# quim0/WFA-GPU

Hardware: AMD Instinct MI355X
Metric: alignments_per_sec (higher is better)
Workload: dtype int32

## Files before the change

### wfa-gpu_amd/csrc/align/cells_hot.inc

```
      typedef __attribute__((address_space(3))) OffT* LdsRow;
      typedef __attribute__((address_space(3))) const uint32_t* LdsWords;
      typedef __attribute__((address_space(1))) uint8_t* GlobalBytes;
      typedef __attribute__((address_space(1))) OffT* GlobalRow;
      OffT* const hm_row0 = Mr + (dm + 2 * de) * rs + kidx0;
      auto hot_cells = [&](const int lo, const int wm1, GlobalBytes& codes, const uint32_t a_oe, const uint32_t a_x, const uint32_t a_m,
                           const uint32_t a_ip, const uint32_t a_ic, const uint32_t d_delta, const uint32_t pw_addr, const uint32_t tw_addr,
                           const uint32_t a_hm, unsigned long long& touch) {
        constexpr int SH = RAW ? 2 : 4, PER = 1 << SH, BITS = RAW ? 3 : 1;
        constexpr uint32_t TB = 16;
        constexpr bool PAIRED = HYBRID || BANDED;
        static_assert(TB >= (uint32_t)PER && (TB & (BT_M_MASK | BT_D_EXT | BT_I_EXT)) == 0, "tag base");
        auto group = [&](const int kq, const GlobalBytes codes, const int left) -> bool {
          bool more_groups;
          const uint32_t vb = (uint32_t)(kq - 1) << 1;
          const int kq16 = kq << 16;
          uint32_t q_mo = vb + a_oe, q_mx = vb + a_x, q_wm = vb + a_m, q_ri = vb + a_ip, q_wi = vb + a_ic;
          uint32_t q_rd = q_ri + d_delta, q_wd = q_wi + d_delta, q_hm = vb + a_hm;
          asm volatile("" : "+v"(q_mo), "+v"(q_mx), "+v"(q_wm), "+v"(q_ri), "+v"(q_wi), "+v"(q_rd), "+v"(q_wd), "+v"(q_hm));
          const LdsRow r_mo = (LdsRow)q_mo, r_mx = (LdsRow)q_mx, w_m = (LdsRow)q_wm;
          const LdsRow r_i = (LdsRow)q_ri, w_i = (LdsRow)q_wi, r_hm = (LdsRow)q_hm;
          auto d_row = [&](const uint32_t q) {
            if constexpr (HYBRID) return (GlobalRow)((GlobalBytes)(uintptr_t)d_first + (ptrdiff_t)(int32_t)q);
            else return (LdsRow)q;
          };
// ... 23 lines not shown
            asm("v_med3_i32 %0, %1, 0, %2" : "=v"(cap) : "v"(mv_t), "n"(PER));
            c.h = mv0;
            c.rem = c.hmax - c.h;
            if constexpr (!RAW) {
              const int vt = mv_t - kq16 - (O << 16);
              asm("v_lshl_add_u32 %0, %1, 2, %2" : "=v"(c.pa) : "v"(vt >> (16 + SH)), "s"(pw_addr));
              asm("v_lshl_add_u32 %0, %1, 2, %2" : "=v"(c.ta) : "v"(mv_t >> (16 + SH)), "s"(tw_addr));
              c.sa = (uint32_t)vt >> 15; c.sb = (uint32_t)mv_t >> 15;
            } else {
              const int v = mv0 - k;
              asm("v_lshl_add_u32 %0, %1, 2, %2" : "=v"(c.pa) : "v"(v >> SH), "s"(pw_addr));
              asm("v_lshl_add_u32 %0, %1, 2, %2" : "=v"(c.ta) : "v"(c.h >> SH), "s"(tw_addr));
              c.sa = (uint32_t)v << BITS; c.sb = (uint32_t)c.h << BITS;
            }
            uint32_t fb;
            {
              const LdsWords pw = (LdsWords)c.pa; const LdsWords tw = (LdsWords)c.ta;
              const uint32_t d0w = __builtin_amdgcn_alignbit(pw[1], pw[0], c.sa) ^ __builtin_amdgcn_alignbit(tw[1], tw[0], c.sb);
              asm("v_ffbl_b32 %0, %1" : "=v"(fb) : "v"(d0w));
            }
            int adv;
            asm("v_min3_i32 %0, %1, %2, %3" : "=v"(adv) : "v"((int)(fb >> BITS)), "v"(c.rem), "v"(cap));
            c.h += adv;
            c.more = adv == PER;
            return c;
          };
          auto back = [&](auto uc, auto partial_tag, const unsigned long long act, ChunkState& c) {
            constexpr int O = decltype(uc)::value * NT;
            constexpr bool PARTIAL = decltype(partial_tag)::value;
            if (__builtin_amdgcn_ballot_w64(c.more) != 0ull) {
              uint32_t fb;
              int togo = c.more ? max(c.rem - PER, 0) : 0;
              while (__builtin_amdgcn_ballot_w64(togo > 0) != 0ull) {
                c.pa += 4; c.ta += 4;
                const LdsWords pw = (LdsWords)c.pa; const LdsWords tw = (LdsWords)c.ta;
                const uint32_t d = __builtin_amdgcn_alignbit(pw[1], pw[0], c.sa) ^ __builtin_amdgcn_alignbit(tw[1], tw[0], c.sb);
                asm("v_ffbl_b32 %0, %1" : "=v"(fb) : "v"(d));
                const int nn = min(min((int)(fb >> BITS), PER), togo);
                c.h += nn;
                togo = (nn == PER) ? togo - PER : 0;
              }
            }
            int mv = c.h, ins_c = c.ins_c, del_t = c.del_t;
            if constexpr (PARTIAL) {
              const bool active = __builtin_amdgcn_inverse_ballot_w64(act);
              mv = active ? c.h : OffNull<OffT>::value;
              ins_c = active ? ins_c : (int)0x80000000u; del_t = active ? del_t : (int)0x80000000u;
            }
            touch |= __builtin_amdgcn_ballot_w64(mv == c.hmax);
            w_m[O + 1] = (OffT)mv;
            w_i[O + 1] = (OffT)(ins_c >> 16);
            w_d[O + 1] = (OffT)(del_t >> 16);
            if constexpr (BT) {
              if constexpr (TILED) codes[(size_t)(t_off + (uint32_t)(O * 4))] = (uint8_t)c.code;
              else codes[O] = (uint8_t)c.code;
            }
          };
          auto chunk = [&](auto uc, auto partial_tag, const unsigned long long act) {
            ChunkState c = front(uc);
            back(uc, partial_tag, act, c);
          };
          auto chunk_pair = [&](auto uc, auto uc2, auto partial2_tag, const unsigned long long act2) {
            ChunkState c0 = front(uc), c1 = front(uc2);
            back(uc, std::false_type{}, 0ull, c0);
            back(uc2, partial2_tag, act2, c1);
          };
          more_groups = false;
          auto from = [&](auto&& self, auto uc) -> void {
            constexpr int Uc = decltype(uc)::value;
            const int n_act = left - Uc * NT;
            if (n_act >= 64) {
              if constexpr (Uc < 3 && PAIRED) {
                const int n2 = n_act - NT;
                if (n2 >= 64) {
                  chunk_pair(uc, std::integral_constant<int, Uc + 1>{}, std::false_type{}, 0ull);
                  if constexpr (Uc + 1 < 3) { if (n2 > NT) self(self, std::integral_constant<int, Uc + 2>{}); }
                  else more_groups = n2 > NT;
                } else if (n2 > 0) {
                  chunk_pair(uc, std::integral_constant<int, Uc + 1>{}, std::true_type{}, (1ull << n2) - 1ull);
                } else {
                  chunk(uc, std::false_type{}, 0ull);
                }
              } else {
              chunk(uc, std::false_type{}, 0ull);
              if constexpr (Uc < 3) { if (n_act > NT) self(self, std::integral_constant<int, Uc + 1>{}); }
              else more_groups = n_act > NT;
              }
            } else if (NW == 1 || n_act > 0) {
              chunk(uc, std::true_type{}, (1ull << n_act) - 1ull);
            }
          };
          from(from, std::integral_constant<int, 0>{});
          return more_groups;
        };
        const int left0 = wm1 + 1 - ((NW == 1) ? 0 : __builtin_amdgcn_readfirstlane(stid & ~63));
        int kq = stid + lo, left = left0;
        if constexpr (NW == 1) {
          if (__builtin_expect(group(kq, codes, left), 0)) {
            constexpr uint32_t STEP = TILED ? 0u : 4u * NT;
            uint32_t adv = 0;
            do { kq += 4 * NT; codes += STEP; adv += STEP; left -= 4 * NT; } while (group(kq, codes, left));
            codes -= adv;
          }
        } else {
          uint32_t adv = 0;
          while (group(kq, codes, left)) { kq += 4 * NT; codes += 4 * NT; adv += 4u * NT; left -= 4 * NT; }
          codes -= adv;
// ... 3 lines not shown
```

### wfa-gpu_amd/csrc/align/loop_lean_any.inc

```
        if constexpr (HOT && !BANDED && !ENDSFREE) {
          if (e != 1 && !touched_ever) {
            const int s_in = s;
            const int o_pen = oe - e;
            int u_w = s_in >= oe ? (s_in - o_pen) / e : 0;
            int g_cnt = s_in >= oe ? e - (s_in - o_pen) % e : oe - s_in;
            int s_clear = INT_MAX;
            if (bounded) {
              const int lo_a = budget - e * (kend - wlo) + 1, lo_b = (budget + o_pen - e * (kend + 1)) / 2 + 1;
              const int hi_a = budget - e * (whi - kend) + 1, hi_b = (budget + o_pen + e * (kend - 1)) / 2 + 1;
              s_clear = min(min(lo_a, lo_b), min(hi_a, hi_b)) - 2 * e - 2;
            }
            s_clear = __builtin_amdgcn_readfirstlane(s_clear);
            const uint32_t rsb = (uint32_t)rs * 2u;
            const uint32_t a_first = lds_addr(m_first), a_end = lds_addr(m_end), ai_first = lds_addr(i_first), ai_end = lds_addr(i_end);
            uint32_t a_m = lds_addr(p_m), a_x = lds_addr(p_x), a_oe = lds_addr(p_oe), a_ic = lds_addr(p_ic), a_ip = lds_addr(p_ip);
            uint32_t d_delta = HYBRID ? 0u - ai_first : (uint32_t)(de * rs) * 2u;
            uint32_t pw_addr = lds_addr(Pw), tw_addr = lds_addr(Tw), a_hm = lds_addr(hm_row0);
            asm volatile("" : "+s"(pw_addr), "+s"(tw_addr), "+s"(a_hm), "+s"(d_delta));
            int lo = last_lo, hi = last_hi;
            int f_lo = max(wlo, rlo), f_hi = min(whi, rhi);
            unsigned long long touch = 0;
            uint32_t a_last = a_m;
            GlobalBytes code_addr = nullptr;
            uint32_t need_prev = 0;
            if constexpr (TILED) code_addr = tile_row(s);
            else if constexpr (BT) code_addr = (GlobalBytes)(uintptr_t)p.arena + ((size_t)chunk_cur * 16u + (uint32_t)stid);
            const uint32_t tile_pitch = tile_cols * 64u - 48u;
            if constexpr (NW > 1) {
              if (tid == 0) { *touch_flag(0) = 0u; *touch_flag(1) = 0u; }
              __syncthreads();
            }
            const bool far_is_oe = oe >= x;
            int why = 0;
            do {
              ++s;
              if (reach_r == 0) { ++rlo; --rhi; reach_r = e - 1; f_lo = max(f_lo, rlo); f_hi = min(f_hi, rhi); } else --reach_r;
              if (--g_cnt == 0) { g_cnt = e; ++u_w; }
              asm volatile("" : "+s"(f_lo), "+s"(f_hi), "+s"(u_w));
              lo = max(-u_w, f_lo); hi = min(u_w, f_hi);
              if (__builtin_expect(lo > hi, 0)) { why = 1; continue; }
              const int wm1 = hi - lo;
              uint32_t need = 0;
              if constexpr (TILED) {
                code_addr += (s & 3) ? 16u : tile_pitch;
              } else if constexpr (BT) {
                need = ((uint32_t)wm1 + 16u) >> 4;
                code_addr += need_prev << 4;
                if (__builtin_expect(need + WFA_ARENA_ROW_SLACK > chunk_left, 0)) {
                  const bool got = refill_arena(need + WFA_ARENA_ROW_SLACK);
                  code_addr = (GlobalBytes)(uintptr_t)cold_params()->arena + ((size_t)chunk_cur * 16u + (uint32_t)stid);
                  need_prev = 0;
                  if (!got) { why = 2; continue; }
                }
              }
              a_m = far_is_oe ? a_oe : a_x;
              a_x += rsb;  if (a_x == a_end) a_x = a_first;
              a_oe += rsb; if (a_oe == a_end) a_oe = a_first;
              a_ic = a_ip;
              a_ip += rsb; if (a_ip == ai_end) a_ip = ai_first;
              ncells += (uint32_t)wm1;
              if constexpr (BT && !TILED) {
                row_s = chunk_cur; chunk_cur += need; chunk_left -= need; need_prev = need;
                if constexpr (NW == 1) {
                  const int sl = s & 63;
                  if (sl == 0) tab[s - 64 + lane] = make_uint2((uint32_t)tabv_row, (uint32_t)tabv_lo);
                  asm("s_mov_b32 m0, %4\n\tv_writelane_b32 %0, %2, m0\n\tv_writelane_b32 %1, %3, m0"
                      : "+v"(tabv_row), "+v"(tabv_lo) : "s"((int)row_s), "s"(lo), "s"(sl));
                } else {
                  if (tid == 0) tab[s] = make_uint2(row_s, (uint32_t)lo);
                }
              }
              if (__builtin_expect(s >= s_clear, 0)) {
                auto clear_guards = [&](const int j0) {
                  const int j = min(j0, 2 * dm - 1);
                  const int q = (j < dm) ? lo - 1 - j : hi + 1 - dm + j;
                  const uint32_t qa = (uint32_t)q << 1;
                  *(LdsRow)(qa + a_m) = (OffT)OffNull<OffT>::value;
                  *(LdsRow)(qa + a_ic) = (OffT)OffNull<OffT>::value;
                  if constexpr (HYBRID) *(GlobalRow)((GlobalBytes)(uintptr_t)d_first + (ptrdiff_t)(int32_t)(qa + a_ic + d_delta)) = (OffT)OffNull<OffT>::value;
                  else *(LdsRow)(qa + a_ic + d_delta) = (OffT)OffNull<OffT>::value;
                };
                clear_guards(tid);
                if constexpr (NW == 1) { if (__builtin_expect(2 * dm > 64, 0)) clear_guards(tid + 64); }
              }
              hot_cells(lo, wm1, code_addr, a_oe, a_x, a_m, a_ip, a_ic, d_delta, pw_addr, tw_addr, a_hm, touch);
              a_last = a_m;
              if constexpr (NW == 1) {
                block_sync<NW>();
                if (touch != 0ull) why = 3;
              } else {
                if (touch != 0ull && lane == 0) atomicOr(touch_flag(s), 1u);
                __syncthreads();
                if (*touch_flag(s) != 0u) why = 3;
              }
            } while (why == 0);
            if constexpr (NW > 1) {
              if (tid < 24) red[tid] = (tid & 7) == 6 ? 0 : (((tid & 7) & 1) ? INT_MIN : INT_MAX);
// ... 35 lines not shown
```

### wfa-gpu_amd/csrc/align/loop_lean_e1.inc

```
        if constexpr (HOT && !BANDED && !ENDSFREE) {
          if (e == 1 && !touched_ever) {
            const int s_in = s, lo_in = last_lo, hi_in = last_hi;
            const int c_lo = bounded ? kend - budget : INT_MIN / 2, c_hi = bounded ? kend + budget : INT_MAX / 2;
            int s_clear = INT_MAX;
            if (bounded) {
              const int t_lo = min(wlo - c_lo, (lo_in + s_in - c_lo) >> 1), t_hi = min(c_hi - whi, (c_hi - hi_in + s_in) >> 1);
              s_clear = min(t_lo, t_hi) - 1;
            }
            s_clear = __builtin_amdgcn_readfirstlane(s_clear);
            const uint32_t rsb = (uint32_t)rs * 2u;
            const uint32_t a_first = lds_addr(m_first), a_end = lds_addr(m_end);
            uint32_t a_m = lds_addr(p_m), a_x = lds_addr(p_x), a_oe = lds_addr(p_oe);
            uint32_t a_ic = lds_addr(p_ic), a_ip = lds_addr(p_ip);
            const uint32_t a_iswap = a_ic ^ a_ip;
            uint32_t d_delta = HYBRID ? 0u - lds_addr(i_first) : (uint32_t)(de * rs) * 2u;
            uint32_t pw_addr = lds_addr(Pw), tw_addr = lds_addr(Tw), a_hm = lds_addr(hm_row0);
            asm volatile("" : "+s"(pw_addr), "+s"(tw_addr), "+s"(a_hm), "+s"(d_delta));
            int lo = lo_in, hi = hi_in;
            int t_lo = s_in + c_lo, t_hi = c_hi - s_in, f_lo = max(wlo, t_lo), f_hi = min(whi, t_hi);
            unsigned long long touch = 0;
            uint32_t a_last = a_m;
            GlobalBytes code_addr = nullptr;
            uint32_t need_prev = 0;
            if constexpr (TILED) code_addr = tile_row(s);
            else if constexpr (BT) code_addr = (GlobalBytes)(uintptr_t)p.arena + ((size_t)chunk_cur * 16u + (uint32_t)stid);
            const uint32_t tile_pitch = tile_cols * 64u - 48u;
            if constexpr (NW > 1) {
              if (tid == 0) { *touch_flag(0) = 0u; *touch_flag(1) = 0u; }
              __syncthreads();
            }
            int why = 0;
            const bool far_is_oe = oe >= x;
            do {
              ++s; ++t_lo; --t_hi;
              f_lo = max(f_lo, t_lo); f_hi = min(f_hi, t_hi);
              asm volatile("" : "+s"(f_lo), "+s"(f_hi));
              lo = max(lo - 1, f_lo); hi = min(hi + 1, f_hi);
              if (__builtin_expect(lo > hi, 0)) { why = 1; continue; }
              const int wm1 = hi - lo;
              uint32_t need = 0;
              if constexpr (TILED) {
                code_addr += (s & 3) ? 16u : tile_pitch;
              } else if constexpr (BT) {
                need = ((uint32_t)wm1 + 16u) >> 4;
                code_addr += need_prev << 4;
                if (__builtin_expect(need + WFA_ARENA_ROW_SLACK > chunk_left, 0)) {
                  const bool got = refill_arena(need + WFA_ARENA_ROW_SLACK);
                  code_addr = (GlobalBytes)(uintptr_t)cold_params()->arena + ((size_t)chunk_cur * 16u + (uint32_t)stid);
                  need_prev = 0;
                  if (!got) { why = 2; continue; }
                }
              }
              a_m = far_is_oe ? a_oe : a_x;
              a_x += rsb;  if (a_x == a_end) a_x = a_first;
              a_oe += rsb; if (a_oe == a_end) a_oe = a_first;
              a_ic ^= a_iswap; a_ip ^= a_iswap;
              ncells += (uint32_t)wm1;
              if constexpr (BT && !TILED) {
                row_s = chunk_cur; chunk_cur += need; chunk_left -= need; need_prev = need;
                if constexpr (NW == 1) {
                  const int sl = s & 63;
                  if (sl == 0) tab[s - 64 + lane] = make_uint2((uint32_t)tabv_row, (uint32_t)tabv_lo);
                  asm("s_mov_b32 m0, %4\n\tv_writelane_b32 %0, %2, m0\n\tv_writelane_b32 %1, %3, m0"
                      : "+v"(tabv_row), "+v"(tabv_lo) : "s"((int)row_s), "s"(lo), "s"(sl));
                } else {
                  if (tid == 0) tab[s] = make_uint2(row_s, (uint32_t)lo);
                }
              }
              if (__builtin_expect(s >= s_clear, 0)) {
                auto clear_guards = [&](const int j0) {
                  const int j = min(j0, 2 * dm - 1);
                  const int q = (j < dm) ? lo - 1 - j : hi + 1 - dm + j;
                  const uint32_t qa = (uint32_t)q << 1;
                  *(LdsRow)(qa + a_m) = (OffT)OffNull<OffT>::value;
                  *(LdsRow)(qa + a_ic) = (OffT)OffNull<OffT>::value;
                  if constexpr (HYBRID) *(GlobalRow)((GlobalBytes)(uintptr_t)d_first + (ptrdiff_t)(int32_t)(qa + a_ic + d_delta)) = (OffT)OffNull<OffT>::value;
                  else *(LdsRow)(qa + a_ic + d_delta) = (OffT)OffNull<OffT>::value;
                };
                clear_guards(tid);
                if constexpr (NW == 1) { if (__builtin_expect(2 * dm > 64, 0)) clear_guards(tid + 64); }
              }
              hot_cells(lo, wm1, code_addr, a_oe, a_x, a_m, a_ip, a_ic, d_delta, pw_addr, tw_addr, a_hm, touch);
              a_last = a_m;
              if constexpr (NW == 1) {
                block_sync<NW>();
                if (touch != 0ull) why = 3;
              } else {
                if (touch != 0ull && lane == 0) atomicOr(touch_flag(s), 1u);
                if constexpr (TIMED) {
                  const bool rec = blockIdx.x == 0 && lane == 0;
                  unsigned long long t_arrive = 0;
                  if (rec) t_arrive = __builtin_amdgcn_s_memtime();
                  __syncthreads();
                  if (rec) {
                    const unsigned long long t_leave = __builtin_amdgcn_s_memtime();
// ... 44 lines not shown
```

### wfa-gpu_amd/csrc/align_kernel.hip

```cpp
#include <type_traits>

#include "wfa_device.h"
#include "pack_device.h"

namespace {

template <typename OffT> struct OffNull { static constexpr int value = -32768; };
template <> struct OffNull<int32_t> { static constexpr int value = INT_MIN / 4; };

template <typename OffT> __device__ __forceinline__ OffT off_store(int v);
template <> __device__ __forceinline__ int16_t off_store<int16_t>(int v) {
  return (int16_t)min(v, 32767);
}
template <> __device__ __forceinline__ int32_t off_store<int32_t>(int v) { return v; }

template <typename T> __device__ __forceinline__ uint32_t lds_addr(const T* p) {
  return (uint32_t)(uintptr_t)(const __attribute__((address_space(3))) void*)p;
}

template <int NW> __device__ __forceinline__ void block_sync() {
  if constexpr (NW == 1) {
    asm volatile("" ::: "memory");
    __builtin_amdgcn_wave_barrier();
  } else {
// ... 247 lines not shown
            cp->score[pair] = -1;
            cp->status[pair] = WFA_ST_ALPHABET;
            if (cp->cells) cp->cells[pair] = 0;
          }
          block_sync<NW>();
          continue;
        }
      } else {
        for (int i = tid; i < pwords; i += NT) Pw[i] = gp[i];
        for (int i = tid; i < twords; i += NT) Tw[i] = gt[i];
      }
      {
        const int cells = (dm + (HYBRID ? 1 : 2) * de + 2 * de2) * rs;
        if constexpr (sizeof(OffT) == 2) {
          uint32_t* w = reinterpret_cast<uint32_t*>(Mr);
          for (int i = tid; i < (cells >> 1); i += NT) w[i] = 0x80008000u;
          if constexpr (HYBRID) {
            uint32_t* wd = reinterpret_cast<uint32_t*>(Dg);
            for (int i = tid; i < ((de * rs) >> 1); i += NT) wd[i] = 0x80008000u;
          }
        } else {
          for (int i = tid; i < cells; i += NT) Mr[i] = (OffT)OffNull<OffT>::value;
        }
        if constexpr (HM_ROW) {
          OffT* hm = Mr + cells;
          for (int i = tid; i < rs; i += NT) hm[i] = (OffT)max(min(plen + (i - kidx0), tlen), 0);
        }
      }
      if constexpr (BOOK_NW == 1) book.reset();
      else { for (int i = tid; i <= bkm; i += NT) { book.A[i] = book.I[i] = book.D[i] = ROW_NONE_A; } }
      if constexpr (TWOPIECE) {
        if constexpr (BOOK_NW == 1) book2.reset();
        else { for (int i = tid; i <= bkm; i += NT) { book2.I[i] = book2.D[i] = ROW_NONE_A; } }
      }
      if constexpr (NW > 1) { if (tid < 24) red[tid] = (tid & 7) == 6 ? 0 : (((tid & 7) & 1) ? INT_MIN : INT_MAX); }
      if constexpr (ADAPTIVE && NW > 1) { if (tid < 6) red2[tid] = (tid & 1) ? INT_MIN : INT_MAX; }
      block_sync<NW>();

      auto refill_arena = [&](const uint32_t units) -> bool {
        ColdParams cp = cold_params();
        const uint32_t grab = max(units, cp->chunk_units);
        uint32_t base = WFA_ROW_NONE;
        if (tid == 0) {
          const unsigned long long b = atomicAdd(cp->arena_top, (unsigned long long)grab);
          if (b + grab <= cp->arena_units) base = (uint32_t)b;
        }
        base = block_bcast<NW>(base, bslot);
        chunk_cur = base; chunk_left = (base == WFA_ROW_NONE) ? 0u : grab;
        return base != WFA_ROW_NONE;
      };
      uint32_t tile_cols = 0;
      GlobalBytes tiles0 = nullptr;
      if constexpr (BT && TILED) {
        tile_cols = (uint32_t)(whi - wlo + 16) >> 4;
        const uint32_t block_units = 4u + 4u * (((uint32_t)budget >> 2) + 1u) * tile_cols + 16u;
        if (chunk_left < block_units + 3u && !refill_arena(block_units + 3u)) status = WFA_ST_NOMEM;
        if (status == WFA_ST_DONE) {
          tab_base = (chunk_cur + 3u) & ~3u;
          chunk_left -= (tab_base - chunk_cur) + block_units; chunk_cur = tab_base + block_units;
          GlobalBytes const blk = (GlobalBytes)(uintptr_t)cold_params()->arena + (size_t)tab_base * 16u;
          if (tid == 0) {
            uint32_t* const hdr = reinterpret_cast<uint32_t*>(p.arena + (size_t)tab_base * 16u);
            hdr[0] = WFA_ROW_NONE; hdr[1] = (uint32_t)wlo; hdr[2] = tile_cols; hdr[3] = (uint32_t)budget;
          }
          tiles0 = blk + 64;
        }
      } else if constexpr (BT) {
        const uint32_t tab_units = (uint32_t)(((long long)budget + 2) >> 1);
        if (chunk_left < tab_units + 1 && !refill_arena(tab_units + 1)) status = WFA_ST_NOMEM;
        if (status == WFA_ST_DONE) {
          tab_base = chunk_cur; row_s = chunk_cur + tab_units; chunk_cur += tab_units + 1; chunk_left -= tab_units + 1;
          tab = reinterpret_cast<uint2*>(p.arena + (size_t)tab_base * 16);
          if (tid == 0) p.arena[(size_t)row_s * 16] = 0;
        }
      }
      auto tile_row = [&](const int sc) -> GlobalBytes { return tiles0 + ((size_t)((uint32_t)sc >> 2) * tile_cols * 64u + ((uint32_t)sc & 3u) * 16u); };
      auto tile_off = [&](const int kk) -> uint32_t { const uint32_t d = (uint32_t)(kk - wlo); return d + 3u * (d & ~15u); };
      uint32_t d0 = 0;
      if constexpr (ENDSFREE) {
        constexpr int SH = RAW ? 2 : 4, PER = 1 << SH, BITS = RAW ? 3 : 1;
        OffT* const row0 = Mr + kidx0;
        const int wave = (NW == 1) ? 0 : __builtin_amdgcn_readfirstlane(tid >> 6);
        for (int k0 = -pbf; k0 <= tbf && end_k == INT_MAX; k0 += NT) {
          const int k = k0 + tid;
          const bool act = k <= tbf;
          int h = max(k, 0), v = h - k;
          int rem = act ? min(plen - v, tlen - h) : 0;
          while (rem > 0) {
            const uint32_t* pw = Pw + (v >> SH); const uint32_t* tw = Tw + (h >> SH);
            const uint32_t d = __builtin_amdgcn_alignbit(pw[1], pw[0], (uint32_t)(v & (PER - 1)) << BITS) ^
                               __builtin_amdgcn_alignbit(tw[1], tw[0], (uint32_t)(h & (PER - 1)) << BITS);
            const int n = min(d ? (int)((uint32_t)__builtin_ctz(d) >> BITS) : PER, rem);
            h += n; v += n; rem -= n;
            if (n < PER) break;
          }
          if (act) row0[k] = (OffT)h;
          const bool hit = act && ((h >= tlen && plen - v <= pef) || (v >= plen && tlen - h <= tef));
          const unsigned long long bh = __builtin_amdgcn_ballot_w64(hit);
          if (bh) end_k = k0 + wave * 64 + (int)__builtin_ctzll(bh);
        }
        if constexpr (NW > 1) {
          if (lane == 0 && end_k != INT_MAX) atomicMin(&red[0], end_k);
          __syncthreads();
          end_k = red[0];
        }
        ncells = (uint32_t)(pbf + tbf + 1);
        book.set(0, pack_range(-pbf, tbf), ROW_NONE_A, ROW_NONE_A);
        done = end_k != INT_MAX;
      }
      if (!ENDSFREE && tid == 0) {
        constexpr int SH = RAW ? 2 : 4, PER = 1 << SH, BITS = RAW ? 3 : 1;
        int h0 = 0, rem = min(plen, tlen);
        while (rem > 0) {
          const uint32_t d = Pw[h0 >> SH] ^ Tw[h0 >> SH];
          const int n = min((int)((d ? (uint32_t)__builtin_ctz(d) : 32u) >> BITS), rem);
          h0 += n; rem -= n;
          if (n < PER) break;
        }
        Mr[kidx0 + GZ] = (OffT)h0;
        d0 = ((kend == 0 && h0 >= tlen) ? 1u : 0u) | (h0 >= min(plen, tlen) ? 2u : 0u);
      }
      if constexpr (!ENDSFREE) {
        book.set(0, pack_range(0, 0), ROW_NONE_A, ROW_NONE_A);
        if constexpr (TWOPIECE) book2.set(0, ROW_NONE_A, ROW_NONE_A);
        d0 = block_bcast<NW>(d0, bslot);
        done = (d0 & 1u) != 0;
      }
      const bool touched_at_0 = (d0 & 2u) != 0;
      block_sync<NW>();
      int steps_wait = 0, null_steps = 0;
// ... 378 lines not shown
```

### wfa-gpu_amd/csrc/trace_kernel.hip

```cpp
#include <cstdlib>
#include <type_traits>

#include "wfa_device.h"
#include "trace_layout.h"

namespace {

#ifdef WFA_TRACE_TWOPIECE_UNIT
constexpr bool TRACE_2P = true;
#else
constexpr bool TRACE_2P = false;
#endif

struct SeqDirect {
  const uint32_t* w;
  __device__ __forceinline__ uint2 pair(int i) const { return make_uint2(w[i], w[i + 1]); }
};
struct SeqWindow {
  static constexpr int WORDS = 8;
  const uint32_t* g;
  int nwords;
  uint32_t* slot;
  int base;
  __device__ __forceinline__ uint2 pair(int i) {
// ... 142 lines not shown
  int v = max(-ends.k0, 0), h = max(ends.k0, 0);
  sink.push_free(ends.k0 > 0 ? 'I' : 'D', (uint32_t)(v + h));
  int n = lcp_seq<RAW>(Pw, Tw, plen, tlen, v, h);
  sink.push('M', (uint32_t)n); v += n; h += n;
  const uint32_t skip = (uint32_t)(reinterpret_cast<uintptr_t>(ops) & 3);
  const uint32_t* ops4 = reinterpret_cast<const uint32_t*>(ops - skip);
  auto op_word = [&](uint32_t idx) -> uint32_t {
    if constexpr (OPS_LDS) return ((const __attribute__((address_space(3))) uint32_t*)ops4)[idx];
    else return ops4[idx];
  };
  uint32_t word = nops ? (op_word(0) >> (8 * skip)) : 0u;
  for (uint32_t i = 0; i < nops; ++i) {
    const uint32_t op = word & 0xFFu;
    if (((i + 1 + skip) & 3u) == 0u) { if (i + 1 < nops) word = op_word((i + 1 + skip) >> 2); } else word >>= 8;
    {
      const uint32_t k3 = op & 3u;
      sink.push(k3 == OP_X ? 'X' : (k3 == OP_I ? 'I' : 'D'), 1);
      v += (k3 != OP_I) ? 1 : 0; h += (k3 != OP_D) ? 1 : 0;
    }
    if (op & OP_EXT_AFTER) {
      n = lcp_seq<RAW>(Pw, Tw, plen, tlen, v, h);
      sink.push('M', (uint32_t)n); v += n; h += n;
    }
  }
  const bool at_end = (h - v == ends.k1) && (v == plen || h == tlen);
  if (at_end) { sink.push_free('D', (uint32_t)(plen - v)); sink.push_free('I', (uint32_t)(tlen - h)); }
  sink.flush();
  if (out && sink.len < out_cap) out[sink.len] = '\0';
  if (cost) *cost = sink.cost;
  return at_end ? sink.len : 0xFFFFFFFFu;
}

template <bool RAW, bool OPS_LDS = false>
__device__ __forceinline__ uint32_t replay(const uint8_t* ops, uint32_t nops, const uint32_t* Pw, const uint32_t* Tw,
                                           int plen, int tlen, const PairEnds ends, char* out, const GapPens pen, int* cost,
                                           uint32_t out_cap = 0xFFFFFFFFu, bool words = false) {
  SeqDirect pv{Pw}, tv{Tw};
  return replay_views<RAW, OPS_LDS>(ops, nops, pv, tv, plen, tlen, ends, out, pen, cost, out_cap, words);
}

constexpr int TRACE_THREADS = 64;

struct BtBlock { const uint8_t* blk; bool tiled; int wlo; uint32_t cols; };
__device__ __forceinline__ BtBlock bt_block(const WfaTraceParams& p, const uint32_t pair) {
  BtBlock b;
  b.blk = p.arena + (size_t)p.bt_final_row[pair] * 16;
  const uint4 hdr = *reinterpret_cast<const uint4*>(b.blk);
  b.tiled = hdr.x == WFA_ROW_NONE; b.wlo = (int)hdr.y; b.cols = hdr.z;
  return b;
}
__device__ __forceinline__ void fetch_bt_rows(const WfaTraceParams& p, const BtBlock& bb, const int sr, const int k, int& kbase, uint8_t* dst) {
  uint4 v0 = make_uint4(0, 0, 0, 0), v1 = make_uint4(0, 0, 0, 0);
  if (bb.tiled) {
    const int c0 = ((k - bb.wlo) - 8) >> 4;
    kbase = bb.wlo + c0 * 16;
    if (sr >= 0) {
      const uint8_t* const row = bb.blk + 64u + (size_t)((uint32_t)sr >> 2) * bb.cols * 64u + ((uint32_t)sr & 3u) * 16u;
      if (c0 >= 0 && (uint32_t)c0 < bb.cols) v0 = *reinterpret_cast<const uint4*>(row + (size_t)c0 * 64u);
      if (c0 + 1 >= 0 && (uint32_t)(c0 + 1) < bb.cols) v1 = *reinterpret_cast<const uint4*>(row + (size_t)(c0 + 1) * 64u);
    }
  } else {
    kbase = k - 8;
    if (sr >= 0) {
      const uint2 row = reinterpret_cast<const uint2*>(bb.blk)[sr];
      const long long off = (long long)row.x * 16 + ((long long)kbase - (int)row.y);
      if (off >= 0 && (unsigned long long)off + 16 <= p.arena_bytes) {
        struct __attribute__((packed, aligned(1))) U16 { uint32_t w[4]; };
        const U16 t = *reinterpret_cast<const U16*>(p.arena + off);
        v0 = make_uint4(t.w[0], t.w[1], t.w[2], t.w[3]);
      }
    }
  }
  reinterpret_cast<uint4*>(dst)[0] = v0;
  reinterpret_cast<uint4*>(dst)[1] = v1;
}

constexpr uint32_t OP_NONE = 0;
__device__ __forceinline__ uint32_t walk_step(const uint32_t code, int& state, int& s, int& k, const WfaTraceParams& p) {
#if defined(WFA_TRACE_LINEAR_UNIT)
  const uint32_t org = code & BTL_MASK;
  if (org == BTL_NONE) return OP_NONE;
  const bool is_x = org == BTL_X, is_d = org == BTL_D;
  s -= is_x ? p.x : p.e;
  k += is_x ? 0 : (is_d ? 1 : -1);
  return (is_x ? OP_X : (is_d ? OP_D : OP_I)) | OP_EXT_AFTER;
#elif defined(WFA_TRACE_TWOPIECE_UNIT)
  uint32_t after = 0;
  int st = state;
  if (st == 0) {
    const uint32_t org = code & BT2_M_MASK;
    if (org == BT2_M_X) { s -= p.x; return OP_X | OP_EXT_AFTER; }
    if (org == BT2_M_NONE || org > BT2_M_X) return OP_NONE;
    st = (int)(org >> 4);
    st = st == 2 ? 3 : (st == 3 ? 2 : st);
    after = OP_EXT_AFTER;
  }
  const bool second = st >= 3, is_d = (st & 1) == 0;
  const uint32_t flag = second ? (is_d ? BT2_D2_EXT : BT2_I2_EXT) : (is_d ? BT2_D1_EXT : BT2_I1_EXT);
  const bool ext = (code & flag) != 0;
  s -= second ? (ext ? p.e2 : p.oe2) : (ext ? p.e : p.oe);
  k += is_d ? 1 : -1;
  state = ext ? st : 0;
  return (is_d ? OP_D : OP_I) | after;
#else
  uint32_t op;
  const bool i_ext = (code & BT_I_EXT) != 0, d_ext = (code & BT_D_EXT) != 0;
  if (state == 0) {
    const uint32_t org = code & BT_M_MASK;
    if (org == BT_M_X) { op = OP_X | OP_EXT_AFTER; s -= p.x; }
    else if (org == BT_M_I) { op = OP_I | OP_EXT_AFTER; --k; s -= i_ext ? p.e : p.oe; state = i_ext ? 1 : 0; }
    else if (org == BT_M_D) { op = OP_D | OP_EXT_AFTER; ++k; s -= d_ext ? p.e : p.oe; state = d_ext ? 2 : 0; }
    else return OP_NONE;
  } else if (state == 1) {
    op = OP_I; --k; s -= i_ext ? p.e : p.oe; state = i_ext ? 1 : 0;
  } else {
    op = OP_D; ++k; s -= d_ext ? p.e : p.oe; state = d_ext ? 2 : 0;
  }
  return op;
#endif
}
struct WalkSpan { int k1, k0_lo, k0_hi; };
__device__ __forceinline__ WalkSpan walk_span(const WfaTraceParams& p, const size_t pair, const int plen, const int tlen) {
  WalkSpan w;
  w.k1 = p.ends ? p.ends[2 * pair + 1] : tlen - plen;
  w.k0_lo = -min(p.span_pbf, plen); w.k0_hi = min(p.span_tbf, tlen);
  return w;
}
__device__ __forceinline__ bool walk_ended(const int s, const int state, const int k, const WalkSpan& w) { return s == 0 && state == 0 && k >= w.k0_lo && k <= w.k0_hi; }
__device__ __forceinline__ PairEnds stored_ends(const WfaTraceParams& p, const size_t pair, const int plen, const int tlen) {
  PairEnds e{0, tlen - plen};
  if (p.ends) { e.k0 = p.ends[2 * pair]; e.k1 = p.ends[2 * pair + 1]; }
  return e;
}

__device__ __forceinline__ void cache_line(const void* line, uint2* const slot) {
  const uint4* src = reinterpret_cast<const uint4*>(line);
  const uint4 a = src[0], b = src[1], c = src[2], d = src[3];
  slot[0] = make_uint2(a.x, a.y); slot[1] = make_uint2(a.z, a.w);
  slot[2] = make_uint2(b.x, b.y); slot[3] = make_uint2(b.z, b.w);
  slot[4] = make_uint2(c.x, c.y); slot[5] = make_uint2(c.z, c.w);
  slot[6] = make_uint2(d.x, d.y); slot[7] = make_uint2(d.z, d.w);
}

__device__ __forceinline__ bool walk_ops(const WfaTraceParams& p, const uint32_t pair, const int score, const int plen, const int tlen,
                                         uint8_t* const q_end, const uint32_t need_ops, uint2* const tab_cache_lane, uint32_t& nops_out, PairEnds& ends_out) {
  bool fail = false;
  uint32_t nops = 0, word = 0;
  const BtBlock bb = bt_block(p, pair);
  const uint2* tab = reinterpret_cast<const uint2*>(bb.blk);
  const WalkSpan span = walk_span(p, pair, plen, tlen);
  int k = span.k1, s = score;
  int state = 0;
  int cached = -1;
  while (s > 0) {
    if (nops >= need_ops) { fail = true; break; }
    uint32_t code;
    if (bb.tiled) {
      const uint32_t d = (uint32_t)(k - bb.wlo);
      if ((d >> 4) >= bb.cols) { fail = true; break; }
      const int tile_id = (int)(((uint32_t)s >> 2) * bb.cols + (d >> 4));
      if (tile_id != cached) { cached = tile_id; cache_line(bb.blk + 64u + (size_t)tile_id * 64u, tab_cache_lane); }
      code = reinterpret_cast<const uint8_t*>(tab_cache_lane)[((uint32_t)s & 3u) * 16u + (d & 15u)];
    } else {
      if ((s >> 3) != cached) { cached = s >> 3; cache_line(tab + (cached << 3), tab_cache_lane); }
      const uint2 row = tab_cache_lane[s & 7];
      code = p.arena[(size_t)row.x * 16 + (uint32_t)(k - (int)row.y)];
    }
    const uint32_t op = walk_step(code, state, s, k, p);
    if (op == OP_NONE) { fail = true; break; }
    word = (word << 8) | op;
    ++nops;
    if ((nops & 3u) == 0u) reinterpret_cast<uint32_t*>(q_end)[-(int)(nops >> 2)] = word;
  }
  if (!walk_ended(s, state, k, span)) fail = true;
  ends_out = PairEnds{k, span.k1};
  if (!fail && p.ends) p.ends[2 * (size_t)pair] = k;
  if (!fail && (nops & 3u)) {
    uint8_t* qq = q_end - (nops & ~3u);
    for (int r = (int)(nops & 3u) - 1; r >= 0; --r) *--qq = (uint8_t)(word >> (8 * r));
  }
  nops_out = nops;
  return !fail;
}

struct PairSeqs {
  int plen, tlen; const uint32_t* P; const uint32_t* T; int raw;
  __device__ __forceinline__ int pwords() const { return (int)trace_seq_words((unsigned)plen, raw != 0); }
  __device__ __forceinline__ int twords() const { return (int)trace_seq_words((unsigned)tlen, raw != 0); }
};
__device__ __forceinline__ PairSeqs pair_seqs(const WfaTraceParams& p, const size_t pair, const int raw) {
  const WfaSeqPair mp = p.meta[pair];
  PairSeqs q;
  q.plen = (int)mp.pattern_len; q.tlen = (int)mp.text_len;
  q.P = p.packed + ((raw ? mp.pattern_offset : mp.pattern_offset_packed) >> 2);
  q.T = p.packed + ((raw ? mp.text_offset : mp.text_offset_packed) >> 2);
  q.raw = raw;
  return q;
}

__device__ __forceinline__ const uint32_t* readlane_ptr(const uint32_t* ptr, const int j) {
  return reinterpret_cast<const uint32_t*>(((unsigned long long)(uint32_t)__builtin_amdgcn_readlane((int)(reinterpret_cast<unsigned long long>(ptr) >> 32), j) << 32) |
                                           (uint32_t)__builtin_amdgcn_readlane((int)reinterpret_cast<unsigned long long>(ptr), j));
}

template <bool OPS_LDS = false, typename PV, typename TV, typename... A>
__device__ __forceinline__ uint32_t replay_any(const int raw, const uint8_t* ops, const uint32_t nops, PV& Pw, TV& Tw, A... a) {
  return raw ? replay_views<true, OPS_LDS>(ops, nops, Pw, Tw, a...) : replay_views<false, OPS_LDS>(ops, nops, Pw, Tw, a...);
}

__device__ __forceinline__ void finish_pair(const WfaTraceParams& p, const size_t pair, const bool fail, const unsigned long long off = 0,
                                            const uint32_t len = 0, const int cost = 0, const int score = 0) {
  if (fail) {
    p.cigar_off[pair] = 0;
    p.cigar_len[pair] = 0xFFFFFFFFu;
    return;
// ... 583 lines not shown
```

### wfa-gpu_amd/csrc/wfa_device.h

```cpp
#pragma once

#include <hip/hip_runtime.h>
#include <hip/hip_ext.h>
#include <stdint.h>

struct WfaSeqPair {
  size_t text_offset;
  size_t pattern_offset;
  size_t text_offset_packed;
  size_t pattern_offset_packed;
  unsigned int text_len;
  unsigned int pattern_len;
  bool has_N;
};
static_assert(sizeof(WfaSeqPair) == 48, "sequence_pair_t ABI");

enum : uint32_t {
  WFA_ST_PENDING = 0,
  WFA_ST_DONE = 1,
  WFA_ST_BAND = 2,
  WFA_ST_SCORE = 3,
  WFA_ST_NOMEM = 4,
  WFA_ST_ALPHABET = 5,
};

enum : uint32_t { BT_M_NONE = 0, BT_M_X = 12, BT_M_D = 8, BT_M_I = 4, BT_M_MASK = 12, BT_D_EXT = 2, BT_I_EXT = 1 };
enum : uint32_t { BT2_M_NONE = 0, BT2_M_X = 5u << 4, BT2_M_D2 = 4u << 4, BT2_M_D1 = 3u << 4, BT2_M_I2 = 2u << 4, BT2_M_I1 = 1u << 4, BT2_M_MASK = 7u << 4,
                  BT2_D2_EXT = 8, BT2_I2_EXT = 4, BT2_D1_EXT = 2, BT2_I1_EXT = 1 };

enum : uint32_t { BTL_NONE = 0, BTL_X = 3, BTL_D = 2, BTL_I = 1, BTL_MASK = 3 };

__host__ __device__ inline long long wfa_gap2p(const long long n, const int oe1, const int e1, const int oe2, const int e2) {
  if (n <= 0) return 0;
  const long long a = oe1 + (n - 1) * e1, b = oe2 + (n - 1) * e2;
  return a < b ? a : b;
}
__host__ __device__ inline long long wfa_reach2p(const long long S, const int oe1, const int e1, const int oe2, const int e2) {
  const long long a = S >= oe1 ? (S - oe1) / e1 + 1 : 0, b = S >= oe2 ? (S - oe2) / e2 + 1 : 0;
  return a > b ? a : b;
}
__host__ __device__ inline int wfa_stray2p(const long long S, const long long ak, const int oe1, const int e1, const int oe2, const int e2) {
  long long lo = 0, hi = wfa_reach2p(S / 2, oe1, e1, oe2, e2);
  while (lo < hi) {
    const long long mid = lo + (hi - lo + 1) / 2;
    if (wfa_gap2p(mid, oe1, e1, oe2, e2) + wfa_gap2p(mid + ak, oe1, e1, oe2, e2) <= S) lo = mid; else hi = mid - 1;
  }
  return (int)lo;
}

enum : uint8_t { OP_X = 1, OP_I = 2, OP_D = 3, OP_EXT_AFTER = 0x10 };

#define WFA_ROW_NONE 0xFFFFFFFFu
constexpr unsigned long long WFA_ARENA_MAX_BYTES = (1ull << 36) - 4096;
static_assert(WFA_ARENA_MAX_BYTES / 16 < WFA_ROW_NONE, "a row unit must never read as the TILES marker");
#define WFA_RING_ROW_PAD 64
#define WFA_ARENA_ROW_SLACK 4u

struct WfaAlignParams {
  const uint32_t* packed;
  const char* ascii;
  unsigned long long* n_raw;
  const WfaSeqPair* meta;
  const uint32_t* work;
  uint32_t n_work;
  const unsigned long long* n_work_dev;
  int only_pending;
  unsigned int* work_counter;
  uint32_t work_shards;
  int x, oe, e;
  int dm, de;
  int book_mask;
  int rs;
  int max_score;
  const int32_t* budget;
  int budget_q, budget_slack, budget_margin;
  int band_width;
  int band_period;
  int seq_words_cap;
  int no_lean;
  int32_t* score;
  uint32_t* status;
  uint32_t* cells;
  unsigned long long* launch_cells;
  unsigned long long* wave_parts;
  uint32_t* fail_list;
  unsigned long long* fail_count;
  int arena_top_known;
  unsigned long long arena_top0_value;
  uint8_t* arena;
  unsigned long long arena_units;
  unsigned long long* arena_top;
  uint32_t chunk_units;
  uint32_t* bt_final_row;
  void* gring;
  int ring16;
  unsigned long long gring_stride;
  unsigned long long* dbg_times;
  uint32_t dbg_cap;
  int span_pbf, span_pef, span_tbf, span_tef;
  int32_t* ends;
  int oe2, e2, de2;
  int ad_min_len, ad_max_dist, ad_steps;
};
constexpr int WFA_LIN_NO_MISMATCH = 1 << 30;

struct WfaTraceParams {
  int raw;
  int seq_lds_stride;
  int emit_pairs;
// ... 98 lines not shown
```

### wfa-gpu_amd/csrc/wfa_host.hip

```cpp
#include <hip/hip_runtime.h>

#include <algorithm>
#include <climits>
#include <cstdio>
#include <cstdlib>
#include <cstring>
#include <vector>

#include "../../include/wfa_gpu_device.h"
#include "wfa_device.h"
#include "trace_layout.h"

static_assert(sizeof(sequence_pair_t) == sizeof(WfaSeqPair), "ABI mirror");

#define HIP_TRY(expr)                                                                   \
  do {                                                                                  \
    hipError_t _e = (expr);                                                             \
    if (_e != hipSuccess) {                                                             \
      fprintf(stderr, "[!] ERROR: HIP %s failed: %s (%s:%d)\n", #expr,                  \
              hipGetErrorString(_e), __FILE__, __LINE__);                               \
      return -1;                                                                        \
    }                                                                                   \
  } while (0)

// ... 652 lines not shown
  if (c->list_b.ensure((size_t)4 * n, st)) return -1;
  if (c->list_c.ensure((size_t)4 * n, st)) return -1;
  if (c->list_d.ensure((size_t)4 * n, st)) return -1;
  if (compute_cigar) {
    if (c->bt_final.ensure((size_t)4 * n, st)) return -1;
    if (c->cig_off[c->out_set].ensure((size_t)8 * n, st)) return -1;
    if (c->cig_len[c->out_set].ensure((size_t)4 * n, st)) return -1;
    if (!c->cig_off[c->out_set ^ 1].p && c->cig_off[c->out_set ^ 1].ensure((size_t)8 * n, st)) return -1;
    if (!c->cig_len[c->out_set ^ 1].p && c->cig_len[c->out_set ^ 1].ensure((size_t)4 * n, st)) return -1;
  }
  const unsigned batch_max_len = std::max(1u, b->max_seq_len);
  unsigned max_len = batch_max_len;
  const int oe = pen.o + pen.e;
  int item_chars = 2;
  for (unsigned v = batch_max_len; v >= 10; v /= 10) ++item_chars;
  item_chars = std::max(item_chars, 6);

  const int extra_items = ef ? 2 : 0;
  if (ef && !d_ends) {
    if (c->ends.ensure((size_t)8 * n, st)) return -1;
    d_ends = static_cast<int32_t*>(c->ends.p);
  }
  WfaAlignParams ap{};
  if (ef) {
    ap.span_pbf = span->pattern_begin_free; ap.span_pef = span->pattern_end_free; ap.span_tbf = span->text_begin_free; ap.span_tef = span->text_end_free;
    ap.ends = d_ends;
  }
  ap.packed = prepacked ? static_cast<const uint32_t*>(b->d_packed) : static_cast<const uint32_t*>(c->packed.p);
  ap.meta = reinterpret_cast<const WfaSeqPair*>(b->d_metadata);
  ap.x = pen.x; ap.oe = oe; ap.e = pen.e;
  ap.dm = std::max(pen.x, oe) + 1;
  ap.de = pen.e + 1;
  if (tp2) { ap.oe2 = o2 + e2; ap.e2 = e2; ap.de2 = e2 + 1; ap.dm = std::max(ap.dm, ap.oe2 + 1); }
  if (lin) { ap.de = 0; ap.dm = (lin_indel ? pen.e : std::max(pen.x, pen.e)) + 1; if (lin_indel) ap.x = WFA_LIN_NO_MISMATCH; }
  if (ad) { ap.ad_min_len = wfad->min_wavefront_length; ap.ad_max_dist = wfad->max_distance_threshold; ap.ad_steps = wfad->steps_between_cutoffs; }
  const int min_op_cost = tp2 ? std::min(pen.x, std::min(pen.e, e2)) : std::min(pen.x, pen.e);
  { int bk = 64; while (bk < ap.dm) bk <<= 1; ap.book_mask = bk - 1; }
  ap.seq_words_cap = (int)((max_len + 15) / 16 + 1);
  ap.score = d_scores;
  ap.status = static_cast<uint32_t*>(c->status.p);
  ap.cells = static_cast<uint32_t*>(c->cells.p);
  ap.work_counter = reinterpret_cast<unsigned int*>(static_cast<char*>(c->counters.p) + CT_BYTES);
  ap.arena_top = ct + CT_ARENA;
  ap.launch_cells = ct + CT_LCELLS;
  ap.no_lean = c->tuning.careful_only ? 1 : 0;
  ap.chunk_units = 256;
  ap.bt_final_row = static_cast<uint32_t*>(c->bt_final.p);

  double est_pair_bytes = 0.25 * ((double)std::min<unsigned>(max_error, 2 * max_len) + 1) * ((double)std::min<unsigned>(max_error, 2 * max_len) + 1) +
                          16.0 * std::min<unsigned>(max_error, 2 * max_len) + 4096.0;
  auto tiled_pair_bytes = [&](const long long B) -> double {
    const int w = window_width(B, pen.o, pen.e, batch_max_len);
    if (w > 1024) return 0.0;
    return 64.0 * (double)((w + 15) / 16) * (double)(B / 4 + 1) + 512.0;
  };
  if (lin) {
    const double B = std::min<unsigned>(max_error, 2 * max_len);
    est_pair_bytes = 0.5 * (B + 1) * (B + 1) / pen.e + 16.0 * B + 4096.0;
  } else if (ad) {
    const double B = std::min<unsigned>(max_error, 2 * max_len);
    est_pair_bytes = (B + 1) * (B + 1) / pen.e + 16.0 * B + 4096.0;
  } else if (!tp2) est_pair_bytes = std::max(est_pair_bytes, tiled_pair_bytes(std::min<long long>(max_error, 2ll * batch_max_len * std::max(pen.x, pen.e))));
  else {
    const double B = std::min<unsigned>(max_error, 2 * max_len);
    est_pair_bytes = 0.5 * (B + 1) * (B + 1) / std::min(pen.e, e2) + 16.0 * B + 4096.0;
  }
  if (ef) {
    const double m = batch_max_len;
    const double start_w = std::min<double>(span->pattern_begin_free, m) + std::min<double>(span->text_begin_free, m) + 1.0;
    est_pair_bytes += start_w * (double)std::min<unsigned>(max_error, 2 * max_len);
  }
  if (compute_cigar) {
    size_t want = c->arena_cfg;
    if (!want) {
      want = (size_t)(est_pair_bytes * 1.1 * n);
      if (want > c->arena.cap) {
        size_t free_b = 0, total_b = 0;
        HIP_TRY(hipMemGetInfo(&free_b, &total_b));
        want = (size_t)std::min<double>((double)want, 0.45 * (double)(free_b + c->arena.cap));
      }
      want = std::max<size_t>(want, (size_t)64 << 20);
      if (c->arena_limit) {
        const double inflight = std::min<double>(n, 2.0 * c->num_cus) * est_pair_bytes * 2.0;
        const size_t lim = std::max<size_t>(c->arena_limit, (size_t)std::min<double>((double)c->arena_limit_max, inflight));
        want = std::min(want, std::max<size_t>(lim, (size_t)64 << 20));
      }
    }
    want = std::min<size_t>(want, (size_t)WFA_ARENA_MAX_BYTES);
    if (c->arena.cap < want && c->arena.ensure(want, st)) return -1;
    ap.arena = static_cast<uint8_t*>(c->arena.p);
    ap.arena_units = c->arena.cap / 16 - 8;
  }

  c->short_ascii_ok = std::max<size_t>(b->sequences_bytes, b->packed_bytes * 4) < ((size_t)1 << 34);
  const bool short_fuses = !ef && !tp2 && !ad && !lin && wfa_short_supported(pen.x, oe, pen.e) && !c->tuning.min_tier && !(compute_cigar && c->tuning.no_short_cigar) && c->short_ascii_ok;
  const bool fused_pack = !prepacked && (b->max_seq_len >= 512u || short_fuses) && !c->tuning.no_fused_pack;
  bool status_unset = prepacked || fused_pack;
  auto ensure_status = [&]() -> int {
    if (status_unset) { HIP_TRY(hipMemsetAsync(c->status.p, 0, (size_t)4 * n, st)); status_unset = false; }
    return 0;
  };
  struct { bool unset; int q, slack, margin; } budget_rule{false, 0, 0, 0};
  unsigned long long cells_host = 0;
  hipEvent_t call_end = c->ev_end;
  bool ct_clean = true;
  if (!c->counters_zeroed) HIP_TRY(hipMemsetAsync(c->counters.p, 0, CT_BYTES + 8 * 64, st));
  else if (c->tuning.verify_counters) {
// ... 581 lines not shown
```

Baseline: 36.35 million.

## Reshape backtrace code tiles from 4x16 to 8x8 scores-by-diagonals

```diff
diff --git a/scratch/tile_model.py b/scratch/tile_model.py
--- /dev/null
+++ b/scratch/tile_model.py
@@ -0,0 +1,83 @@
+#!/usr/bin/env python3
+import argparse
+import os
+import re
+import sys
+
+import numpy as np
+
+ROOT = os.path.dirname(os.path.dirname(os.path.abspath(__file__)))
+sys.path.insert(0, os.path.join(ROOT, "wfa-gpu_amd", "bindings"))
+sys.path.insert(0, os.path.join(ROOT, "tests"))
+
+SHAPES = [(4, 16), (8, 8), (16, 4), (8, 16), (16, 8)]
+
+
+def cells_read(cigar, score, k_end, pen):
+    x, o, e = pen
+    ops = []
+    for n, c in re.findall(r"(\d*)([MXID])", cigar):
+        ops += [c] * (int(n) if n else 1)
+    s, k = score, k_end
+    out = []
+    i = len(ops) - 1
+    while i >= 0:
+        c = ops[i]
+        if c == "M":
+            i -= 1
+            continue
+        if c == "X":
+            out.append((s, k))
+            s -= x
+            i -= 1
+            continue
+        j = i
+        while j >= 0 and ops[j] == c:
+            j -= 1
+        n = i - j
+        for b in range(n):
+            out.append((s, k))
+            s -= (o + e) if b == n - 1 else e
+            k += -1 if c == "I" else 1
+        i = j
+    assert s == 0 and k == 0, (s, k)
+    return out
+
+
+def main():
+    ap = argparse.ArgumentParser()
+    ap.add_argument("--pairs", type=int, default=4096)
+    ap.add_argument("--length", type=int, default=1000)
+    ap.add_argument("--error", type=float, default=0.05)
+    ap.add_argument("--pen", default="2,3,1")
+    ap.add_argument("--seed", type=int, default=1000)
+    a = ap.parse_args()
+    pen = tuple(int(v) for v in a.pen.split(","))
+    import oracle_lib
+    import wfagpu
+    if not os.path.exists(oracle_lib.ORACLE_SO):
+        oracle_lib.build()
+    buf, meta = wfagpu.generate_pairs(a.pairs, a.length, a.error, seed=a.seed)
+    scores, cigars, _ = oracle_lib.oracle_batch(buf, meta, pen, cigar=True, nthreads=min(16, os.cpu_count() or 1))
+    wlo = -1024
+    lines = {sh: 0 for sh in SHAPES}
+    reads = 0
+    for i in range(a.pairs):
+        k_end = int(meta["text_len"][i]) - int(meta["pattern_len"][i])
+        cells = cells_read(cigars[i], int(scores[i]), k_end, pen)
+        reads += len(cells)
+        sk = np.array(cells, dtype=np.int64).reshape(-1, 2)
+        for ts, tk in SHAPES:
+            tid = (sk[:, 0] // ts) * (1 << 20) + (sk[:, 1] - wlo) // tk
+            n = int(len(tid) > 0) + int(np.count_nonzero(tid[1:] != tid[:-1]))
+            lines[(ts, tk)] += n * max(1, ts * tk // 64)
+    print(f"{a.pairs} pairs of {a.length} bp at {a.error:g}, penalties {pen}, oracle CIGARs: mean score {scores.mean():.1f}, "
+          f"{reads / a.pairs:.1f} origin bytes read per alignment")
+    print("tile (scores x diagonals) | bytes | tiles touched per alignment | 64-byte lines per alignment")
+    for ts, tk in SHAPES:
+        per = lines[(ts, tk)] / a.pairs
+        print(f"{ts:2d} x {tk:2d} | {ts * tk:3d} | {per / max(1, ts * tk // 64):6.2f} | {per:6.2f}")
+
+
+if __name__ == "__main__":
+    main()
diff --git a/wfa-gpu_amd/csrc/align/cells_hot.inc b/wfa-gpu_amd/csrc/align/cells_hot.inc
--- a/wfa-gpu_amd/csrc/align/cells_hot.inc
+++ b/wfa-gpu_amd/csrc/align/cells_hot.inc
@@ -99,7 +99,7 @@
             w_i[O + 1] = (OffT)(ins_c >> 16);
             w_d[O + 1] = (OffT)(del_t >> 16);
             if constexpr (BT) {
-              if constexpr (TILED) codes[(size_t)(t_off + (uint32_t)(O * 4))] = (uint8_t)c.code;
+              if constexpr (TILED) codes[(size_t)(t_off + (uint32_t)(O / 64) * WFA_TILE_CHUNK_BYTES)] = (uint8_t)c.code;
               else codes[O] = (uint8_t)c.code;
             }
           };
diff --git a/wfa-gpu_amd/csrc/align/loop_lean_any.inc b/wfa-gpu_amd/csrc/align/loop_lean_any.inc
--- a/wfa-gpu_amd/csrc/align/loop_lean_any.inc
+++ b/wfa-gpu_amd/csrc/align/loop_lean_any.inc
@@ -25,7 +25,7 @@
             uint32_t need_prev = 0;
             if constexpr (TILED) code_addr = tile_row(s);
             else if constexpr (BT) code_addr = (GlobalBytes)(uintptr_t)p.arena + ((size_t)chunk_cur * 16u + (uint32_t)stid);
-            const uint32_t tile_pitch = tile_cols * 64u - 48u;
+            const uint32_t tile_pitch = wfa_tile_group_pitch(tile_cols);
             if constexpr (NW > 1) {
               if (tid == 0) { *touch_flag(0) = 0u; *touch_flag(1) = 0u; }
               __syncthreads();
@@ -42,7 +42,7 @@
               const int wm1 = hi - lo;
               uint32_t need = 0;
               if constexpr (TILED) {
-                code_addr += (s & 3) ? 16u : tile_pitch;
+                code_addr += (s & (int)(WFA_TILE_TS - 1u)) ? WFA_TILE_TK : tile_pitch;
               } else if constexpr (BT) {
                 need = ((uint32_t)wm1 + 16u) >> 4;
                 code_addr += need_prev << 4;
diff --git a/wfa-gpu_amd/csrc/align/loop_lean_e1.inc b/wfa-gpu_amd/csrc/align/loop_lean_e1.inc
--- a/wfa-gpu_amd/csrc/align/loop_lean_e1.inc
+++ b/wfa-gpu_amd/csrc/align/loop_lean_e1.inc
@@ -24,7 +24,7 @@
             uint32_t need_prev = 0;
             if constexpr (TILED) code_addr = tile_row(s);
             else if constexpr (BT) code_addr = (GlobalBytes)(uintptr_t)p.arena + ((size_t)chunk_cur * 16u + (uint32_t)stid);
-            const uint32_t tile_pitch = tile_cols * 64u - 48u;
+            const uint32_t tile_pitch = wfa_tile_group_pitch(tile_cols);
             if constexpr (NW > 1) {
               if (tid == 0) { *touch_flag(0) = 0u; *touch_flag(1) = 0u; }
               __syncthreads();
@@ -40,7 +40,7 @@
               const int wm1 = hi - lo;
               uint32_t need = 0;
               if constexpr (TILED) {
-                code_addr += (s & 3) ? 16u : tile_pitch;
+                code_addr += (s & (int)(WFA_TILE_TS - 1u)) ? WFA_TILE_TK : tile_pitch;
               } else if constexpr (BT) {
                 need = ((uint32_t)wm1 + 16u) >> 4;
                 code_addr += need_prev << 4;
diff --git a/wfa-gpu_amd/csrc/align_kernel.hip b/wfa-gpu_amd/csrc/align_kernel.hip
--- a/wfa-gpu_amd/csrc/align_kernel.hip
+++ b/wfa-gpu_amd/csrc/align_kernel.hip
@@ -323,18 +323,19 @@
       uint32_t tile_cols = 0;
       GlobalBytes tiles0 = nullptr;
       if constexpr (BT && TILED) {
-        tile_cols = (uint32_t)(whi - wlo + 16) >> 4;
-        const uint32_t block_units = 4u + 4u * (((uint32_t)budget >> 2) + 1u) * tile_cols + 16u;
-        if (chunk_left < block_units + 3u && !refill_arena(block_units + 3u)) status = WFA_ST_NOMEM;
+        tile_cols = wfa_tile_cols((uint32_t)(whi - wlo + 1));
+        const uint32_t block_units = wfa_tile_block_units(tile_cols, (uint32_t)budget);
+        constexpr uint32_t AL = WFA_TILE_UNITS - 1u;
+        if (chunk_left < block_units + AL && !refill_arena(block_units + AL)) status = WFA_ST_NOMEM;
         if (status == WFA_ST_DONE) {
-          tab_base = (chunk_cur + 3u) & ~3u;
+          tab_base = (chunk_cur + AL) & ~AL;
           chunk_left -= (tab_base - chunk_cur) + block_units; chunk_cur = tab_base + block_units;
           GlobalBytes const blk = (GlobalBytes)(uintptr_t)cold_params()->arena + (size_t)tab_base * 16u;
           if (tid == 0) {
             uint32_t* const hdr = reinterpret_cast<uint32_t*>(p.arena + (size_t)tab_base * 16u);
             hdr[0] = WFA_ROW_NONE; hdr[1] = (uint32_t)wlo; hdr[2] = tile_cols; hdr[3] = (uint32_t)budget;
           }
-          tiles0 = blk + 64;
+          tiles0 = blk + WFA_TILE_HEADER_BYTES;
         }
       } else if constexpr (BT) {
         const uint32_t tab_units = (uint32_t)(((long long)budget + 2) >> 1);
@@ -345,8 +346,10 @@
           if (tid == 0) p.arena[(size_t)row_s * 16] = 0;
         }
       }
-      auto tile_row = [&](const int sc) -> GlobalBytes { return tiles0 + ((size_t)((uint32_t)sc >> 2) * tile_cols * 64u + ((uint32_t)sc & 3u) * 16u); };
-      auto tile_off = [&](const int kk) -> uint32_t { const uint32_t d = (uint32_t)(kk - wlo); return d + 3u * (d & ~15u); };
+      auto tile_row = [&](const int sc) -> GlobalBytes {
+        return tiles0 + ((size_t)((uint32_t)sc / WFA_TILE_TS) * tile_cols * WFA_TILE_BYTES + ((uint32_t)sc & (WFA_TILE_TS - 1u)) * WFA_TILE_TK);
+      };
+      auto tile_off = [&](const int kk) -> uint32_t { return wfa_tile_off((uint32_t)(kk - wlo)); };
       uint32_t d0 = 0;
       if constexpr (ENDSFREE) {
         constexpr int SH = RAW ? 2 : 4, PER = 1 << SH, BITS = RAW ? 3 : 1;
diff --git a/wfa-gpu_amd/csrc/trace_kernel.hip b/wfa-gpu_amd/csrc/trace_kernel.hip
--- a/wfa-gpu_amd/csrc/trace_kernel.hip
+++ b/wfa-gpu_amd/csrc/trace_kernel.hip
@@ -218,13 +218,25 @@
 __device__ __forceinline__ void fetch_bt_rows(const WfaTraceParams& p, const BtBlock& bb, const int sr, const int k, int& kbase, uint8_t* dst) {
   uint4 v0 = make_uint4(0, 0, 0, 0), v1 = make_uint4(0, 0, 0, 0);
   if (bb.tiled) {
-    const int c0 = ((k - bb.wlo) - 8) >> 4;
-    kbase = bb.wlo + c0 * 16;
+    constexpr int TK = (int)WFA_TILE_TK, NC = TILE_LDS_W / TK;
+    static_assert(TILE_LDS_W == 32 && TILE_LDS_W % TK == 0, "a row of the LDS tile is two uint4");
+    const int c0 = ((k - bb.wlo) - (TILE_LDS_W - TK) / 2) >> __builtin_ctz(WFA_TILE_TK);
+    kbase = bb.wlo + c0 * TK;
+    uint32_t w[TILE_LDS_W / 4] = {};
     if (sr >= 0) {
-      const uint8_t* const row = bb.blk + 64u + (size_t)((uint32_t)sr >> 2) * bb.cols * 64u + ((uint32_t)sr & 3u) * 16u;
-      if (c0 >= 0 && (uint32_t)c0 < bb.cols) v0 = *reinterpret_cast<const uint4*>(row + (size_t)c0 * 64u);
-      if (c0 + 1 >= 0 && (uint32_t)(c0 + 1) < bb.cols) v1 = *reinterpret_cast<const uint4*>(row + (size_t)(c0 + 1) * 64u);
-    }
+      const uint8_t* const row = bb.blk + WFA_TILE_HEADER_BYTES + (size_t)((uint32_t)sr / WFA_TILE_TS) * bb.cols * WFA_TILE_BYTES + ((uint32_t)sr & (WFA_TILE_TS - 1u)) * WFA_TILE_TK;
+#pragma unroll
+      for (int j = 0; j < NC; ++j) {
+        const int c = c0 + j;
+        if (c >= 0 && (uint32_t)c < bb.cols) {
+          const uint8_t* const src = row + (size_t)c * WFA_TILE_BYTES;
+          if constexpr (TK == 16) { const uint4 t = *reinterpret_cast<const uint4*>(src); w[4 * j] = t.x; w[4 * j + 1] = t.y; w[4 * j + 2] = t.z; w[4 * j + 3] = t.w; }
+          else if constexpr (TK == 8) { const uint2 t = *reinterpret_cast<const uint2*>(src); w[2 * j] = t.x; w[2 * j + 1] = t.y; }
+          else { w[j] = *reinterpret_cast<const uint32_t*>(src); }
+        }
+      }
+    }
+    v0 = make_uint4(w[0], w[1], w[2], w[3]); v1 = make_uint4(w[4], w[5], w[6], w[7]);
   } else {
     kbase = k - 8;
     if (sr >= 0) {
@@ -322,11 +334,12 @@
     if (nops >= need_ops) { fail = true; break; }
     uint32_t code;
     if (bb.tiled) {
+      static_assert(WFA_TILE_BYTES == 64, "cache_line copies one 64-byte tile into the lane's slot");
       const uint32_t d = (uint32_t)(k - bb.wlo);
-      if ((d >> 4) >= bb.cols) { fail = true; break; }
-      const int tile_id = (int)(((uint32_t)s >> 2) * bb.cols + (d >> 4));
-      if (tile_id != cached) { cached = tile_id; cache_line(bb.blk + 64u + (size_t)tile_id * 64u, tab_cache_lane); }
-      code = reinterpret_cast<const uint8_t*>(tab_cache_lane)[((uint32_t)s & 3u) * 16u + (d & 15u)];
+      if (d / WFA_TILE_TK >= bb.cols) { fail = true; break; }
+      const int tile_id = (int)(((uint32_t)s / WFA_TILE_TS) * bb.cols + d / WFA_TILE_TK);
+      if (tile_id != cached) { cached = tile_id; cache_line(bb.blk + WFA_TILE_HEADER_BYTES + (size_t)tile_id * WFA_TILE_BYTES, tab_cache_lane); }
+      code = reinterpret_cast<const uint8_t*>(tab_cache_lane)[((uint32_t)s & (WFA_TILE_TS - 1u)) * WFA_TILE_TK + (d & (WFA_TILE_TK - 1u))];
     } else {
       if ((s >> 3) != cached) { cached = s >> 3; cache_line(tab + (cached << 3), tab_cache_lane); }
       const uint2 row = tab_cache_lane[s & 7];
diff --git a/wfa-gpu_amd/csrc/wfa_device.h b/wfa-gpu_amd/csrc/wfa_device.h
--- a/wfa-gpu_amd/csrc/wfa_device.h
+++ b/wfa-gpu_amd/csrc/wfa_device.h
@@ -55,6 +55,24 @@
 static_assert(WFA_ARENA_MAX_BYTES / 16 < WFA_ROW_NONE, "a row unit must never read as the TILES marker");
 #define WFA_RING_ROW_PAD 64
 #define WFA_ARENA_ROW_SLACK 4u
+
+constexpr uint32_t WFA_TILE_TS = 8;
+constexpr uint32_t WFA_TILE_TK = 8;
+constexpr uint32_t WFA_TILE_BYTES = WFA_TILE_TS * WFA_TILE_TK;
+constexpr uint32_t WFA_TILE_UNITS = WFA_TILE_BYTES / 16;
+constexpr uint32_t WFA_TILE_HEADER_BYTES = 64;
+constexpr uint32_t WFA_TILE_CHUNK_BYTES = 64 * WFA_TILE_TS;
+constexpr uint32_t WFA_TILE_SLACK_TILES = 64 / WFA_TILE_TK;
+static_assert((WFA_TILE_TS & (WFA_TILE_TS - 1)) == 0 && (WFA_TILE_TK & (WFA_TILE_TK - 1)) == 0, "tile sides are powers of two");
+static_assert(WFA_TILE_TK >= 4 && WFA_TILE_TK <= 16 && WFA_TILE_BYTES == 64,
+              "the readers: fetch_bt_rows loads 4, 8 or 16 bytes of a tile row at once, walk_ops keeps one 64-byte tile per lane (LANE_CACHE_BYTES)");
+__host__ __device__ constexpr uint32_t wfa_tile_cols(const uint32_t width) { return (width - 1u + WFA_TILE_TK) / WFA_TILE_TK; }
+__host__ __device__ constexpr uint32_t wfa_tile_groups(const uint32_t budget) { return budget / WFA_TILE_TS + 1u; }
+__host__ __device__ constexpr uint32_t wfa_tile_block_units(const uint32_t cols, const uint32_t budget) {
+  return WFA_TILE_HEADER_BYTES / 16 + WFA_TILE_UNITS * (wfa_tile_groups(budget) * cols + WFA_TILE_SLACK_TILES);
+}
+__host__ __device__ constexpr uint32_t wfa_tile_off(const uint32_t d) { return d + (WFA_TILE_TS - 1u) * (d & ~(WFA_TILE_TK - 1u)); }
+__host__ __device__ constexpr uint32_t wfa_tile_group_pitch(const uint32_t cols) { return cols * WFA_TILE_BYTES - (WFA_TILE_TS - 1u) * WFA_TILE_TK; }
 
 struct WfaAlignParams {
   const uint32_t* packed;
diff --git a/wfa-gpu_amd/csrc/wfa_host.hip b/wfa-gpu_amd/csrc/wfa_host.hip
--- a/wfa-gpu_amd/csrc/wfa_host.hip
+++ b/wfa-gpu_amd/csrc/wfa_host.hip
@@ -728,7 +728,7 @@
   auto tiled_pair_bytes = [&](const long long B) -> double {
     const int w = window_width(B, pen.o, pen.e, batch_max_len);
     if (w > 1024) return 0.0;
-    return 64.0 * (double)((w + 15) / 16) * (double)(B / 4 + 1) + 512.0;
+    return 16.0 * (double)(wfa_tile_block_units(wfa_tile_cols((uint32_t)std::max(w, 1)), (uint32_t)std::max<long long>(B, 0)) + WFA_TILE_UNITS - 1u);
   };
   if (lin) {
     const double B = std::min<unsigned>(max_error, 2 * max_len);
```

Result: no change. 36.68 million, median of 6 (+0.9%).
